# robflynnyh/long-context-asr

Measured on AMD Instinct MI355X. Metric: spectrogram-frames/sec (6L/768D, seq=16384), higher is better.
Workload: dtype bf16; 1 GPU; 6L/768D/6H SConformerXL, seq=16384, rotary theta=1.5M, fwd+CTC+bwd+clip+MADGRAD; per_gpu_batch=128, global_batch=128, seq_len=16384, parallelism=dp1

## Files before the change

long-context-asr_amd/csrc/subsample_mfma.hip:

```cpp
#include "common.h"

namespace {

constexpr int PK = 16;
constexpr int PPOS = 64;
constexpr int PATCH_BYTES = (PPOS + 1) * PK * 2;

__device__ __forceinline__ unsigned pack2(float a, float b) {
    bf16x2 t = {(bf16)a, (bf16)b};
    return __builtin_bit_cast(unsigned, t);
}
__device__ __forceinline__ float dot2(unsigned a, unsigned b, float c) {
    return __builtin_amdgcn_fdot2_f32_bf16(__builtin_bit_cast(bf16x2, a), __builtin_bit_cast(bf16x2, b), c, false);
}

template <typename TX> struct PatchEntry {
    float v0, v1;
    __device__ __forceinline__ void fetch(const TX* __restrict__ xb, int F, int T, int F2, int T2, int t2, int idx) {
        const int pos = idx >> 3, kp = idx & 7;
        const bool row_ok = t2 >= 0 && t2 < T2 && pos < F2;
        float v[2];
#pragma unroll
        for (int e = 0; e < 2; ++e) {
            const int k = 2 * kp + e, kc = min(k, 8);
            const int a = kc / 3, b = kc - 3 * a, t = 2 * t2 + a - 1, f = 2 * pos + b - 1;
            const float m = ld_f(xb + (long)min(max(f, 0), F - 1) * T + min(max(t, 0), T - 1));
            const float tap = (row_ok && t >= 0 && t < T && f >= 0 && f < F) ? m : 0.f;
            const float one = row_ok ? 1.f : 0.f;
            v[e] = k < 9 ? tap : (k < 11 ? one : 0.f);
        }
        v0 = v[0]; v1 = v[1];
    }
    __device__ __forceinline__ void store(char* patch, int idx) const {
        *reinterpret_cast<unsigned*>(patch + (idx >> 3) * (PK * 2) + (idx & 7) * 4) = pack2(v0, v1);
    }
};

__device__ __forceinline__ bf16x8 w0_frag(const float* __restrict__ w0g, const float* __restrict__ b0g, int c, int hh) {
    bf16x8 f;
    const float bias = b0g[c];
    const bf16 bh = (bf16)bias;
#pragma unroll
    for (int j = 0; j < 8; ++j) {
        const int k = 8 * hh + j;
        float v = 0.f;
        if (k < 9) v = w0g[c * 9 + min(k, 8)];
        else if (k == 9) v = (float)bh;
        else if (k == 10) v = bias - (float)bh;
        f[j] = (bf16)v;
    }
    return f;
}

template <typename TX, int NCB>
__global__ __launch_bounds__(512, (NCB == 1 ? 4 : 2)) void stage01_fwd_mfma_kernel(const TX* __restrict__ x, const float* __restrict__ w0g, const float* __restrict__ b0g,
                                                                  const float* __restrict__ wdg, const float* __restrict__ bdg, bf16* __restrict__ d1,
                                                                  int F, int T, int C, int Cs, int T2, int F2, int T4, int F4, int rows_per_block) {
    extern __shared__ __attribute__((aligned(16))) char smem[];
    const int cbase = blockIdx.z * Cs, Cl = min(Cs, C - cbase);
    w0g += cbase * 9; b0g += cbase; wdg += cbase * 9; bdg += cbase; d1 += cbase;
    const int NPAIR = F2 / 2 + 2, QS = 4 * Cl + 128, SLOT = NPAIR * QS;
    char* patch = smem;
    char* act = smem + 2 * PATCH_BYTES;
    const int tid = threadIdx.x, lane = tid & 63, wave = tid >> 6, hh = lane >> 5, cl = lane & 31;
    const int b = blockIdx.y;
    const TX* xb = x + (long)b * F * T;
    const int ncb = Cl / 32;

    bf16x8 wf[NCB];
    unsigned wj0[NCB][3][2], wj12[NCB][3][2];
    float bd2[NCB][2];
    const int cp = lane & 15, fg = lane >> 4;
#pragma unroll
    for (int u = 0; u < NCB; ++u) {
        const int cb = min(wave + 8 * u, ncb - 1);
        wf[u] = w0_frag(w0g, b0g, cb * 32 + cl, hh);
#pragma unroll
        for (int ch = 0; ch < 2; ++ch) {
            const int c = cb * 32 + 2 * cp + ch;
            bd2[u][ch] = bdg[c];
#pragma unroll
            for (int i = 0; i < 3; ++i) { wj0[u][i][ch] = pack2(0.f, wdg[c * 9 + 3 * i]); wj12[u][i][ch] = pack2(wdg[c * 9 + 3 * i + 1], wdg[c * 9 + 3 * i + 2]); }
        }
    }
    for (int i = tid; i < 3 * (QS / 4); i += 512) *reinterpret_cast<unsigned*>(act + (i / (QS / 4)) * SLOT + (i % (QS / 4)) * 4) = 0u;
    if (tid < 2 * PK / 2) *reinterpret_cast<unsigned*>(patch + (tid / (PK / 2)) * PATCH_BYTES + PPOS * PK * 2 + (tid % (PK / 2)) * 4) = 0u;

    const int r0 = blockIdx.x * rows_per_block, r1 = min(T4, r0 + rows_per_block);
    const int t2_first = 2 * r0 - 1, t2_last = 2 * (r1 - 1) + 1;
    PatchEntry<TX> pe, pe2;
    pe.fetch(xb, F, T, F2, T2, t2_first, tid);
    pe.store(patch, tid);
    pe.fetch(xb, F, T, F2, T2, t2_first + 1, tid);
    __syncthreads();
    for (int t2 = t2_first; t2 <= t2_last; ++t2) {
        const int buf = (t2 - t2_first) & 1;
        const char* pcur = patch + buf * PATCH_BYTES;
        if (t2 + 1 < t2_last) pe2.fetch(xb, F, T, F2, T2, t2 + 2, tid);
        char* arow = act + ((t2 + 3) % 3) * SLOT;
#pragma unroll
        for (int u = 0; u < NCB; ++u) {
            if (wave + 8 * u >= ncb) break;
            const int c = (wave + 8 * u) * 32 + cl;
#pragma unroll
            for (int blk = 0; blk < 2; ++blk) {
                if (blk * 32 >= F2) break;
                const bf16x8 a = *reinterpret_cast<const bf16x8*>(pcur + (blk * 32 + cl) * (PK * 2) + hh * 16);
                f32x16 acc;
#pragma unroll
                for (int r = 0; r < 16; ++r) acc[r] = 0.f;
                acc = __builtin_amdgcn_mfma_f32_32x32x16_bf16(a, wf[u], acc, 0, 0, 0);
#pragma unroll
                for (int g = 0; g < 8; ++g) {
                    const int f2 = blk * 32 + acc_row(2 * g, hh), q = (f2 + 2) >> 1;
                    if (q < NPAIR)
                        *reinterpret_cast<unsigned*>(arow + q * QS + c * 4) = pack2(siluf_(acc[2 * g]), siluf_(acc[2 * g + 1]));
                }
            }
        }
        if (t2 < t2_last) pe.store(patch + (buf ^ 1) * PATCH_BYTES, tid);
        pe = pe2;
        __syncthreads();
        if ((t2 & 1) == 0) continue;
        const int t4 = (t2 - 1) >> 1;
        if (t4 < r0) continue;
#pragma unroll
        for (int u = 0; u < NCB; ++u) {
            if (wave + 8 * u >= ncb) break;
            const int c0 = (wave + 8 * u) * 32 + 2 * cp;
#pragma unroll
            for (int fi = 0; fi < 8; ++fi) {
                const int f4 = fg + 4 * fi;
                if (f4 >= F4) break;
                float a0 = bd2[u][0], a1 = bd2[u][1];
#pragma unroll
                for (int i = 0; i < 3; ++i) {
                    const char* srow = act + ((2 * t4 + i - 1 + 3) % 3) * SLOT + c0 * 4;
                    const uint2 pa = *reinterpret_cast<const uint2*>(srow + f4 * QS);
                    const uint2 pb = *reinterpret_cast<const uint2*>(srow + (f4 + 1) * QS);
                    a0 = dot2(pa.x, wj0[u][i][0], a0); a0 = dot2(pb.x, wj12[u][i][0], a0);
                    a1 = dot2(pa.y, wj0[u][i][1], a1); a1 = dot2(pb.y, wj12[u][i][1], a1);
                }
                *reinterpret_cast<unsigned*>(d1 + (((long)b * T4 + t4) * F4 + f4) * C + c0) = pack2(a0, a1);
            }
        }
        __syncthreads();
    }
}

template <int NCB>
__global__ __launch_bounds__(512, 4) void dwconv_window_fwd_kernel(const bf16* __restrict__ x, const float* __restrict__ wdg, const float* __restrict__ bdg,
                                                                   bf16* __restrict__ y, int Ti, int Fi, int C, int To, int Fo, int rows_per_block) {
    extern __shared__ __attribute__((aligned(16))) char smem[];
    const int NPAIR = Fi / 2 + 2, QS = 4 * C + 128, SLOT = NPAIR * QS;
    char* act = smem;
    const int tid = threadIdx.x, lane = tid & 63, wave = tid >> 6;
    const int b = blockIdx.y, ncb = C / 32;
    const bf16* xb = x + (long)b * Ti * Fi * C;
    unsigned wj0[NCB][3][2], wj12[NCB][3][2];
    float bd2[NCB][2];
    const int cp = lane & 15, fg = lane >> 4;
#pragma unroll
    for (int u = 0; u < NCB; ++u) {
        const int cb = min(wave + 8 * u, ncb - 1);
#pragma unroll
        for (int ch = 0; ch < 2; ++ch) {
            const int c = cb * 32 + 2 * cp + ch;
            bd2[u][ch] = bdg[c];
#pragma unroll
            for (int i = 0; i < 3; ++i) { wj0[u][i][ch] = pack2(0.f, wdg[c * 9 + 3 * i]); wj12[u][i][ch] = pack2(wdg[c * 9 + 3 * i + 1], wdg[c * 9 + 3 * i + 2]); }
        }
    }
    for (int i = tid; i < 3 * (QS / 4); i += 512) *reinterpret_cast<unsigned*>(act + (i / (QS / 4)) * SLOT + (i % (QS / 4)) * 4) = 0u;

    const int npq = (Fi + 1) / 2, items = npq * (C / 8);
    struct Row { bf16x8 a[2], b[2]; };
    auto fetch = [&](Row& r, int ti) {
        const bool row_ok = ti >= 0 && ti < Ti;
        const bf16* src = xb + (long)min(max(ti, 0), Ti - 1) * Fi * C;
        const bf16x8 z = {0, 0, 0, 0, 0, 0, 0, 0};
#pragma unroll
        for (int it = 0; it < 2; ++it) {
            const int idx = min(tid + 512 * it, items - 1), q = idx / (C / 8), c8 = idx - q * (C / 8);
            const bf16x8 va = *reinterpret_cast<const bf16x8*>(src + (long)(2 * q) * C + c8 * 8);
            const bf16x8 vb = *reinterpret_cast<const bf16x8*>(src + (long)min(2 * q + 1, Fi - 1) * C + c8 * 8);
            r.a[it] = row_ok ? va : z;
            r.b[it] = (row_ok && 2 * q + 1 < Fi) ? vb : z;
        }
    };
    auto produce = [&](const Row& r, int ti) {
        char* arow = act + ((ti + 3) % 3) * SLOT;
#pragma unroll
        for (int it = 0; it < 2; ++it) {
            const int idx = tid + 512 * it;
            if (idx < items) {
                const int q = idx / (C / 8), c8 = idx - q * (C / 8);
                unsigned w[8];
#pragma unroll
                for (int e = 0; e < 8; ++e) w[e] = pack2(siluf_((float)r.a[it][e]), siluf_((float)r.b[it][e]));
                uint4* d = reinterpret_cast<uint4*>(arow + (q + 1) * QS + c8 * 32);
                d[0] = make_uint4(w[0], w[1], w[2], w[3]); d[1] = make_uint4(w[4], w[5], w[6], w[7]);
            }
        }
    };

    const int r0 = blockIdx.x * rows_per_block, r1 = min(To, r0 + rows_per_block);
    const int ti_first = 2 * r0 - 1, ti_last = 2 * (r1 - 1) + 1;
    Row row;
    fetch(row, ti_first);
    __syncthreads();
    for (int ti = ti_first; ti <= ti_last; ++ti) {
        produce(row, ti);
        if (ti < ti_last) fetch(row, ti + 1);
        __syncthreads();
        if ((ti & 1) == 0) continue;
        const int to = (ti - 1) >> 1;
        if (to < r0) continue;
#pragma unroll
        for (int u = 0; u < NCB; ++u) {
            if (wave + 8 * u >= ncb) break;
            const int c0 = (wave + 8 * u) * 32 + 2 * cp;
            for (int fo = fg; fo < Fo; fo += 4) {
                float a0 = bd2[u][0], a1 = bd2[u][1];
#pragma unroll
                for (int i = 0; i < 3; ++i) {
                    const char* srow = act + ((2 * to + i - 1 + 3) % 3) * SLOT + c0 * 4;
                    const uint2 pa = *reinterpret_cast<const uint2*>(srow + fo * QS);
                    const uint2 pb = *reinterpret_cast<const uint2*>(srow + (fo + 1) * QS);
                    a0 = dot2(pa.x, wj0[u][i][0], a0); a0 = dot2(pb.x, wj12[u][i][0], a0);
                    a1 = dot2(pa.y, wj0[u][i][1], a1); a1 = dot2(pb.y, wj12[u][i][1], a1);
                }
                *reinterpret_cast<unsigned*>(y + (((long)b * To + to) * Fo + fo) * C + c0) = pack2(a0, a1);
            }
        }
        __syncthreads();
    }
}

template <typename TX, int NCB>
__global__ __launch_bounds__(512, (NCB == 1 ? 4 : 2)) void stage01_bwd_mfma_kernel(const TX* __restrict__ x, const float* __restrict__ w0g, const float* __restrict__ b0g,
                                                                  const float* __restrict__ wdg, const bf16* __restrict__ dd1,
                                                                  float* __restrict__ dw0, float* __restrict__ db0, float* __restrict__ dwd, float* __restrict__ dbd,
                                                                  int F, int T, int C, int Cs, int T2, int F2, int T4, int F4, int rows_per_block,
                                                                  long det_stride) {
    extern __shared__ __attribute__((aligned(16))) char smem[];
    const int cbase = blockIdx.z * Cs, Cl = min(Cs, C - cbase);
    {
        const long drow = ((long)blockIdx.y * gridDim.x + blockIdx.x) * det_stride;
        dw0 += drow + cbase * 9; db0 += drow + cbase; dwd += drow + cbase * 9; dbd += drow + cbase;
    }
    w0g += cbase * 9; b0g += cbase; wdg += cbase * 9;
    const int GS = 2 * Cl, GSLOT = (F4 + 2) * GS;
    char* patch = smem;
    char* gimg = smem + 2 * PATCH_BYTES;
    const int tid = threadIdx.x, lane = tid & 63, wave = tid >> 6, hh = lane >> 5, cl = lane & 31;
    const int b = blockIdx.y;
    const TX* xb = x + (long)b * F * T;
    const bf16* gb = dd1 + (long)b * T4 * F4 * C + cbase;
    const int ncb = Cl / 32;

    const bool qtaps = gridDim.z > 1;
    bf16x8 wf[NCB];
    float wd[NCB][9], gwd[NCB][9], gbd[NCB];
    f32x16 aw0[NCB];
#pragma unroll
    for (int u = 0; u < NCB; ++u) {
        const int c = min(wave + 8 * u, ncb - 1) * 32 + cl;
        wf[u] = w0_frag(w0g, b0g, c, hh);
        gbd[u] = 0.f;
#pragma unroll
        for (int k = 0; k < 9; ++k) { const float w = wdg[c * 9 + k]; wd[u][k] = qtaps ? (float)(bf16)w : w; gwd[u][k] = 0.f; }
#pragma unroll
        for (int r = 0; r < 16; ++r) aw0[u][r] = 0.f;
    }
    if (tid < 2 * PK / 2) *reinterpret_cast<unsigned*>(patch + (tid / (PK / 2)) * PATCH_BYTES + PPOS * PK * 2 + (tid % (PK / 2)) * 4) = 0u;

    for (int i = tid; i < 3 * GSLOT / 4; i += 512) *reinterpret_cast<unsigned*>(gimg + i * 4) = 0u;
    __syncthreads();
    const unsigned lds_g = __builtin_amdgcn_readfirstlane(lds_addr(gimg));
    const int gseg = Cl / 8, gchunks = F4 * gseg;
    auto gissue = [&](int to) {
        if (to < 0 || to >= T4) return;
        const bf16* src = gb + (long)to * F4 * C;
        const unsigned dst = lds_g + (unsigned)((to & 1) * GSLOT) + (unsigned)__builtin_amdgcn_readfirstlane(tid & ~63) * 16u;
        for (int i = 0; i * 512 < gchunks; ++i) {
            const int ch = tid + 512 * i;
            if (ch < gchunks) dma16_asm(src + (long)(ch / gseg) * C + (ch % gseg) * 8, dst + (unsigned)(i * 512 * 16));
        }
    };

    const int r0 = blockIdx.x * rows_per_block, r1 = min(T2, r0 + rows_per_block);
    PatchEntry<TX> pe, pe2;
    pe.fetch(xb, F, T, F2, T2, r0, tid);
    gissue(r0 >> 1);
    pe.store(patch, tid);
    pe.fetch(xb, F, T, F2, T2, r0 + 1, tid);
    wait_vm<0>();
    __syncthreads();
    for (int t2 = r0; t2 < r1; ++t2) {
        const int buf = (t2 - r0) & 1;
        const char* pcur = patch + buf * PATCH_BYTES;
        const bool odd = t2 & 1;
        if (t2 + 2 < r1) pe2.fetch(xb, F, T, F2, T2, t2 + 2, tid);
        if (!odd) gissue((t2 >> 1) + 1);
        const int toX = (odd ? t2 + 1 : t2) >> 1, toZ = (t2 - 1) >> 1;
        const char* gX = gimg + (toX < T4 ? (toX & 1) : 2) * GSLOT;
        const char* gZ = gimg + (toZ & 1) * GSLOT;
#pragma unroll
        for (int u = 0; u < NCB; ++u) {
            if (wave + 8 * u >= ncb) break;
            const int c = (wave + 8 * u) * 32 + cl;
#pragma unroll 1
            for (int blk = 0; blk < 2; ++blk) {
                if (blk * 32 >= F2) break;
                const bf16x8 a = *reinterpret_cast<const bf16x8*>(pcur + (blk * 32 + cl) * (PK * 2) + hh * 16);
                f32x16 pre;
#pragma unroll
                for (int r = 0; r < 16; ++r) pre[r] = 0.f;
                pre = __builtin_amdgcn_mfma_f32_32x32x16_bf16(a, wf[u], pre, 0, 0, 0);
                unsigned dpk[8];
#pragma unroll
                for (int g4 = 0; g4 < 4; ++g4) {
                    const int base = blk * 32 + 8 * g4 + 4 * hh, p = base >> 2;
                    if (base >= F2) { dpk[2 * g4] = 0u; dpk[2 * g4 + 1] = 0u; continue; }
                    float sg[4], sv[4], gs[4];
#pragma unroll
                    for (int e = 0; e < 4; ++e) { const float v = pre[4 * g4 + e]; sg[e] = sigmoidf_(v); sv[e] = v * sg[e]; gs[e] = 0.f; }
                    auto taps = [&](const char* grow, int i) {
                        const unsigned short* gp_ = reinterpret_cast<const unsigned short*>(grow + (2 * p) * GS + c * 2);
                        const float g0 = __builtin_bit_cast(float, (unsigned)gp_[0] << 16);
                        const float g1 = __builtin_bit_cast(float, (unsigned)gp_[Cl] << 16);
                        const float g2 = __builtin_bit_cast(float, (unsigned)gp_[2 * Cl] << 16);
                        const float* w = wd[u] + 3 * i;
                        float* gw = gwd[u] + 3 * i;
                        gs[0] += w[1] * g0;                 gw[1] += g0 * sv[0];
                        gs[1] += w[0] * g1 + w[2] * g0;     gw[0] += g1 * sv[1]; gw[2] += g0 * sv[1];
                        gs[2] += w[1] * g1;                 gw[1] += g1 * sv[2];
                        gs[3] += w[0] * g2 + w[2] * g1;     gw[0] += g2 * sv[3]; gw[2] += g1 * sv[3];
                        if (i == 1) gbd[u] += g0 + g1;
                    };
                    if (!odd) taps(gX, 1);
                    else { taps(gX, 0); taps(gZ, 2); }
                    float d4[4];
#pragma unroll
                    for (int e = 0; e < 4; ++e) {
                        const float v = pre[4 * g4 + e];
                        const float d = gs[e] * sg[e] * (1.f + v * (1.f - sg[e]));
                        d4[e] = (base + e < F2) ? d : 0.f;
                    }
                    dpk[2 * g4] = pack2(d4[0], d4[1]); dpk[2 * g4 + 1] = pack2(d4[2], d4[3]);
                    __builtin_amdgcn_sched_barrier(0);
                }
                {
                    const int i16 = lane & 15, q4 = i16 >> 2, p4 = i16 & 3, G = (lane >> 4) & 1;
                    const char* tb = pcur + (blk * 32 + 4 * hh + q4) * (PK * 2) + G * 32 + (p4 >> 1) * 16 + (p4 & 1) * 8;
#pragma unroll
                    for (int half = 0; half < 2; ++half) {
                        if (blk * 32 + 16 * half >= F2) break;
                        const bf16x4 lo = __builtin_amdgcn_ds_read_tr16_b64_v4bf16((lds_p4)(tb + (16 * half) * (PK * 2)));
                        const bf16x4 hi = __builtin_amdgcn_ds_read_tr16_b64_v4bf16((lds_p4)(tb + (16 * half + 8) * (PK * 2)));
                        const bf16x8 at = __builtin_shufflevector(lo, hi, 0, 1, 2, 3, 4, 5, 6, 7);
                        const uint4 bw = make_uint4(dpk[4 * half], dpk[4 * half + 1], dpk[4 * half + 2], dpk[4 * half + 3]);
                        aw0[u] = __builtin_amdgcn_mfma_f32_32x32x16_bf16(at, __builtin_bit_cast(bf16x8, bw), aw0[u], 0, 0, 0);
                    }
                }
            }
        }
        if (t2 + 1 < r1) pe.store(patch + (buf ^ 1) * PATCH_BYTES, tid);
        pe = pe2;
        wait_vm<0>();
        __syncthreads();
    }
#pragma unroll
    for (int u = 0; u < NCB; ++u) {
        if (wave + 8 * u >= ncb) break;
        const int c = (wave + 8 * u) * 32 + cl;
#pragma unroll
        for (int r = 0; r < 4; ++r) atomicAdd(dw0 + c * 9 + 4 * hh + r, aw0[u][r]);
        if (hh == 0) { atomicAdd(dw0 + c * 9 + 8, aw0[u][4]); atomicAdd(db0 + c, aw0[u][5]); }
#pragma unroll
        for (int k = 0; k < 9; ++k) { const float v = gwd[u][k] + __shfl_xor(gwd[u][k], 32, 64); if (hh == 0) atomicAdd(dwd + c * 9 + k, v); }
        const float v = gbd[u] + __shfl_xor(gbd[u], 32, 64);
        if (hh == 0) atomicAdd(dbd + c, v);
    }
}

}

static size_t stage01_fwd_lds(int F2, long cs) { return 2 * (size_t)PATCH_BYTES + 3 * (size_t)(F2 / 2 + 2) * (4 * cs + 128); }
static size_t stage01_bwd_lds(int F4, long cs) { return 2 * (size_t)PATCH_BYTES + 3 * (size_t)(F4 + 2) * 2 * cs; }
constexpr size_t FWD_LDS_MAX = 160 * 1024, BWD_LDS_MAX = 80 * 1024;

static int stage01_slab_channels(long F, long C, bool bwd) {
    const int F2 = conv_out(F), F4 = conv_out(F2);
    if (C <= 0 || C % 32 != 0 || C > 1024 || F2 > PPOS) return 0;
    if (sub_mfma_off()) return 0;
    auto fits = [&](long cs) { return bwd ? stage01_bwd_lds(F4, cs) <= BWD_LDS_MAX : stage01_fwd_lds(F2, cs) <= FWD_LDS_MAX; };
    if (C <= 512) return fits(C) ? (int)C : 0;
    long cs = 256;
    if (const char* e = getenv("SCONF_SUB_SLAB")) { const long v = atol(e); if (v >= 32 && v <= 512 && v % 32 == 0) cs = v; }
    while (cs > 32 && !fits(cs)) cs -= 32;
    return fits(cs) ? (int)cs : 0;
}
int stage01_mfma_slabs(int64_t F, int64_t C, int bwd) {
    const int cs = stage01_slab_channels(F, C, bwd != 0);
    return cs ? (int)cdiv(C, (long)cs) : 0;
}

int sconf_stage01_fwd_mfma(const void* x, int x_dtype, const float* w0, const float* b0, const float* wd, const float* bd, void* d1,
                           int64_t B, int64_t F, int64_t T, int64_t C, hipStream_t stream) {
    const int T2 = conv_out(T), F2 = conv_out(F), T4 = conv_out(T2), F4 = conv_out(F2);
    const int Cs = stage01_slab_channels(F, C, false);
    if (!Cs) return 0;
    const size_t sh = stage01_fwd_lds(F2, Cs);
    const long target = env_long("SCONF_SUB_FWD_BLOCKS", 4096);
    const int rpb = std::max(1, (int)cdiv((long)T4 * B, target));
    dim3 grid(cdiv(T4, rpb), (unsigned)B, (unsigned)cdiv(C, (long)Cs)), block(512);
#define LF(TX, NCB_) do { \
        static bool attr = false; lds_limit_once(attr, {(const void*)stage01_fwd_mfma_kernel<TX, NCB_>}, FWD_LDS_MAX); \
        hipLaunchKernelGGL((stage01_fwd_mfma_kernel<TX, NCB_>), grid, block, sh, stream, (const TX*)x, w0, b0, wd, bd, (bf16*)d1, (int)F, (int)T, (int)C, Cs, T2, F2, T4, F4, rpb); } while (0)
    if (x_dtype == SCONF_F32) { if (Cs <= 256) LF(float, 1); else LF(float, 2); }
    else                      { if (Cs <= 256) LF(bf16, 1); else LF(bf16, 2); }
#undef LF
    return 1;
}

static bool stage01_bwd_mfma_geo(long B, long F, long T, long C, dim3& grid, size_t& sh, int& rpb, int& Cs) {
    const int T2 = conv_out(T), F2 = conv_out(F), F4 = conv_out(F2);
    Cs = stage01_slab_channels(F, C, true);
    if (!Cs) return false;
    sh = stage01_bwd_lds(F4, Cs);
    const long target = env_long("SCONF_SUB_BWD_BLOCKS", 2048);
    rpb = std::max(2, (int)cdiv((long)T2 * B, target));
    rpb += rpb & 1;
    grid = dim3(cdiv(T2, rpb), (unsigned)B, (unsigned)cdiv(C, (long)Cs));
    return true;
}
int64_t stage01_bwd_mfma_workspace(int64_t B, int64_t F, int64_t T, int64_t C) {
    dim3 grid; size_t sh; int rpb, Cs;
    if (B * T * F == 0 || !stage01_bwd_mfma_geo(B, F, T, C, grid, sh, rpb, Cs)) return 0;
    return (int64_t)grid.x * grid.y * 20 * C * 4;
}

int sconf_stage01_bwd_mfma(const void* dd1, const void* x, int x_dtype, const float* w0, const float* b0, const float* wd,
                           float* dw0, float* db0, float* dwd, float* dbd, void* workspace, int64_t workspace_bytes,
                           int64_t B, int64_t F, int64_t T, int64_t C, hipStream_t stream) {
    const int T2 = conv_out(T), F2 = conv_out(F), T4 = conv_out(T2), F4 = conv_out(F2);
    dim3 grid; size_t sh; int rpb, Cs;
    if (!stage01_bwd_mfma_geo(B, F, T, C, grid, sh, rpb, Cs)) return 0;
    const dim3 block(512);
    const long rows = (long)grid.x * grid.y, dst = 20 * C;
    float* sl = det_begin<float>(workspace, workspace_bytes, rows, dst, stream);
    if (!sl) { sconf_set_error("sconf_sub_stage01_bwd: needs %ld bytes of workspace (sconf_sub_stage01_bwd_workspace)", rows * dst * 4); return -1; }
#define LB(TX, NCB_) do { \
        if (sh > 64 * 1024) { static bool attr = false; lds_limit_once(attr, {(const void*)stage01_bwd_mfma_kernel<TX, NCB_>}, BWD_LDS_MAX); } \
        hipLaunchKernelGGL((stage01_bwd_mfma_kernel<TX, NCB_>), grid, block, sh, stream, (const TX*)x, w0, b0, wd, (const bf16*)dd1, sl, sl + 9 * C, sl + 10 * C, sl + 19 * C, (int)F, (int)T, (int)C, Cs, T2, F2, T4, F4, rpb, dst); } while (0)
    if (x_dtype == SCONF_F32) { if (Cs <= 256) LB(float, 1); else LB(float, 2); }
    else                      { if (Cs <= 256) LB(bf16, 1); else LB(bf16, 2); }
#undef LB
    det_finish<float>(sl, rows, dst, DetSegs<float>{{dw0, db0, dwd, dbd}, {0, 9 * C, 10 * C, 19 * C}, {9 * C, C, 9 * C, C}, 4}, stream);
    return 1;
}

int sconf_dwconv_window_fwd(const void* x, const float* w, const float* bias, void* y, int64_t B, int64_t Ti, int64_t Fi, int64_t C, hipStream_t stream) {
    const int To = conv_out(Ti), Fo = conv_out(Fi);
    if (C % 32 != 0 || C > 512 || ((Fi + 1) / 2) * (C / 8) > 1024) return 0;
    if (sub_mfma_off()) return 0;
    const size_t sh = 3 * (size_t)(Fi / 2 + 2) * (4 * C + 128);
    if (sh > 160 * 1024) return 0;
    const long target = env_long("SCONF_SUB_FWD_BLOCKS", 4096);
    const int rpb = std::max(1, (int)cdiv((long)To * B, target));
    dim3 grid(cdiv(To, rpb), (unsigned)B), block(512);
#define LW(NCB_) do { \
        static bool attr = false; lds_limit_once(attr, {(const void*)dwconv_window_fwd_kernel<NCB_>}, 160 * 1024); \
        hipLaunchKernelGGL((dwconv_window_fwd_kernel<NCB_>), grid, block, sh, stream, (const bf16*)x, w, bias, (bf16*)y, (int)Ti, (int)Fi, (int)C, To, Fo, rpb); } while (0)
    if (C <= 256) LW(1); else LW(2);
#undef LW
    return 1;
}
```

Before: 7.124 million spectrogram-frames/sec.

## Batch patch fetches by R rows and per-wave dd1 DMA layout in subsample bwd

The stage0/1 backward kernel now fetches input patches for R conv0 rows at once into a double set of R patch buffers. It synchronises once per group instead of once per row, with a partial vmcnt wait so the dd1 DMA for the next row can stay in flight. The gradient image in LDS is changed to per-wave 32-channel bins so each wave issues its own DMA, and patch fetches now keep raw inputs in registers and convert them at store time. The kernel also gains optional timestamp instrumentation, and the LDS footprint grows with R.

```diff
diff --git a/long-context-asr_amd/csrc/subsample_mfma.hip b/long-context-asr_amd/csrc/subsample_mfma.hip
--- a/long-context-asr_amd/csrc/subsample_mfma.hip
+++ b/long-context-asr_amd/csrc/subsample_mfma.hip
@@ -1,6 +1,29 @@
+#ifdef SCONF_SUB_STAMP
+#define SCONF_STAMPS
+#endif
 #include "common.h"
 
 namespace {
+
+#ifdef SCONF_SUB_STAMP
+__device__ unsigned long long g_sub_stamps[2 * 8 * 8];
+#define STAMP_OUT(k) do { if (blockIdx.x == gridDim.x / 2 && blockIdx.y == gridDim.y / 2 && blockIdx.z == 0 && (threadIdx.x & 63) == 0) \
+        for (int i_ = 0; i_ < 8; ++i_) g_sub_stamps[((k) * 8 + (threadIdx.x >> 6)) * 8 + i_] = st_acc_[i_]; } while (0)
+static void sub_stamp_print(int k, double rows, hipStream_t stream, const char* legend) {
+    if (!getenv("SCONF_SUB_STAMP_PRINT")) return;
+    (void)hipStreamSynchronize(stream);
+    unsigned long long h[2 * 8 * 8];
+    (void)hipMemcpyFromSymbol(h, HIP_SYMBOL(g_sub_stamps), sizeof(h));
+    for (int w = 0; w < 8; ++w) {
+        fprintf(stderr, "[stage01 %s stamps] wave %d:", k ? "bwd" : "fwd", w);
+        double tot = 0;
+        for (int i = 0; i < 8; ++i) { fprintf(stderr, " %7.1f", (double)h[(k * 8 + w) * 8 + i] / rows); tot += (double)h[(k * 8 + w) * 8 + i] / rows; }
+        fprintf(stderr, "  sum %7.1f   (memtime ticks per conv0 row over %.0f rows: %s)\n", tot, rows, legend);
+    }
+}
+#else
+#define STAMP_OUT(k)
+#endif
 
 constexpr int PK = 16;
 constexpr int PPOS = 64;
@@ -15,26 +38,39 @@
 }
 
 template <typename TX> struct PatchEntry {
-    float v0, v1;
-    __device__ __forceinline__ void fetch(const TX* __restrict__ xb, int F, int T, int F2, int T2, int t2, int idx) {
-        const int pos = idx >> 3, kp = idx & 7;
-        const bool row_ok = t2 >= 0 && t2 < T2 && pos < F2;
+    TX r0, r1;
+    int t2;
+    static __device__ __forceinline__ void tap_of(int t2, int idx, int e, int& k, int& t, int& f) {
+        k = 2 * (idx & 7) + e;
+        const int kc = min(k, 8), a = kc / 3, b = kc - 3 * a;
+        t = 2 * t2 + a - 1; f = 2 * (idx >> 3) + b - 1;
+    }
+    __device__ __forceinline__ void fetch(const TX* __restrict__ xb, int F, int T, int t2_, int idx) {
+        int k, t, f;
+        t2 = t2_;
+        tap_of(t2, idx, 0, k, t, f); r0 = xb[(long)min(max(f, 0), F - 1) * T + min(max(t, 0), T - 1)];
+        tap_of(t2, idx, 1, k, t, f); r1 = xb[(long)min(max(f, 0), F - 1) * T + min(max(t, 0), T - 1)];
+    }
+    __device__ __forceinline__ void store(char* patch, int F, int T, int F2, int T2, int idx) const {
+        const bool row_ok = t2 >= 0 && t2 < T2 && (idx >> 3) < F2;
         float v[2];
 #pragma unroll
         for (int e = 0; e < 2; ++e) {
-            const int k = 2 * kp + e, kc = min(k, 8);
-            const int a = kc / 3, b = kc - 3 * a, t = 2 * t2 + a - 1, f = 2 * pos + b - 1;
-            const float m = ld_f(xb + (long)min(max(f, 0), F - 1) * T + min(max(t, 0), T - 1));
+            int k, t, f;
+            tap_of(t2, idx, e, k, t, f);
+            const float m = (float)(e ? r1 : r0);
             const float tap = (row_ok && t >= 0 && t < T && f >= 0 && f < F) ? m : 0.f;
             const float one = row_ok ? 1.f : 0.f;
             v[e] = k < 9 ? tap : (k < 11 ? one : 0.f);
         }
-        v0 = v[0]; v1 = v[1];
-    }
-    __device__ __forceinline__ void store(char* patch, int idx) const {
-        *reinterpret_cast<unsigned*>(patch + (idx >> 3) * (PK * 2) + (idx & 7) * 4) = pack2(v0, v1);
+        *reinterpret_cast<unsigned*>(patch + (idx >> 3) * (PK * 2) + (idx & 7) * 4) = pack2(v[0], v[1]);
     }
 };
+
+__device__ __forceinline__ float dp_of(float gs, float sg, float pre) {
+#pragma clang fp reassociate(off)
+    return ((1.f + pre * (1.f - sg)) * sg) * gs;
+}
 
 __device__ __forceinline__ bf16x8 w0_frag(const float* __restrict__ w0g, const float* __restrict__ b0g, int c, int hh) {
     bf16x8 f;
@@ -89,14 +125,16 @@
     const int r0 = blockIdx.x * rows_per_block, r1 = min(T4, r0 + rows_per_block);
     const int t2_first = 2 * r0 - 1, t2_last = 2 * (r1 - 1) + 1;
     PatchEntry<TX> pe, pe2;
-    pe.fetch(xb, F, T, F2, T2, t2_first, tid);
-    pe.store(patch, tid);
-    pe.fetch(xb, F, T, F2, T2, t2_first + 1, tid);
+    pe.fetch(xb, F, T, t2_first, tid);
+    pe.store(patch, F, T, F2, T2, tid);
+    pe.fetch(xb, F, T, t2_first + 1, tid);
     __syncthreads();
+    STAMP_DECL(8)
     for (int t2 = t2_first; t2 <= t2_last; ++t2) {
         const int buf = (t2 - t2_first) & 1;
         const char* pcur = patch + buf * PATCH_BYTES;
-        if (t2 + 1 < t2_last) pe2.fetch(xb, F, T, F2, T2, t2 + 2, tid);
+        if (t2 + 1 < t2_last) pe2.fetch(xb, F, T, t2 + 2, tid);
+        STAMP(0);
         char* arow = act + ((t2 + 3) % 3) * SLOT;
 #pragma unroll
         for (int u = 0; u < NCB; ++u) {
@@ -118,9 +156,12 @@
                 }
             }
         }
-        if (t2 < t2_last) pe.store(patch + (buf ^ 1) * PATCH_BYTES, tid);
+        STAMP(2);
+        if (t2 < t2_last) pe.store(patch + (buf ^ 1) * PATCH_BYTES, F, T, F2, T2, tid);
         pe = pe2;
+        STAMP(3);
         __syncthreads();
+        STAMP(5);
         if ((t2 & 1) == 0) continue;
         const int t4 = (t2 - 1) >> 1;
         if (t4 < r0) continue;
@@ -144,8 +185,11 @@
                 *reinterpret_cast<unsigned*>(d1 + (((long)b * T4 + t4) * F4 + f4) * C + c0) = pack2(a0, a1);
             }
         }
+        STAMP(6);
         __syncthreads();
-    }
+        STAMP(7);
+    }
+    STAMP_OUT(0);
 }
 
 template <int NCB>
@@ -237,7 +281,7 @@
     }
 }
 
-template <typename TX, int NCB>
+template <typename TX, int NCB, int R>
 __global__ __launch_bounds__(512, (NCB == 1 ? 4 : 2)) void stage01_bwd_mfma_kernel(const TX* __restrict__ x, const float* __restrict__ w0g, const float* __restrict__ b0g,
                                                                   const float* __restrict__ wdg, const bf16* __restrict__ dd1,
                                                                   float* __restrict__ dw0, float* __restrict__ db0, float* __restrict__ dwd, float* __restrict__ dbd,
@@ -250,9 +294,11 @@
         dw0 += drow + cbase * 9; db0 += drow + cbase; dwd += drow + cbase * 9; dbd += drow + cbase;
     }
     w0g += cbase * 9; b0g += cbase; wdg += cbase * 9;
-    const int GS = 2 * Cl, GSLOT = (F4 + 2) * GS;
+    static_assert(R >= 2 && R % 2 == 0, "a group starts on an even conv0 row");
+    const int GBIN = 64, GCB = (F4 + 2) * GBIN;
+    const int GSLOT = (Cl / 32) * GCB;
     char* patch = smem;
-    char* gimg = smem + 2 * PATCH_BYTES;
+    char* gimg = smem + 2 * R * PATCH_BYTES;
     const int tid = threadIdx.x, lane = tid & 63, wave = tid >> 6, hh = lane >> 5, cl = lane & 31;
     const int b = blockIdx.y;
     const TX* xb = x + (long)b * F * T;
@@ -273,43 +319,59 @@
 #pragma unroll
         for (int r = 0; r < 16; ++r) aw0[u][r] = 0.f;
     }
-    if (tid < 2 * PK / 2) *reinterpret_cast<unsigned*>(patch + (tid / (PK / 2)) * PATCH_BYTES + PPOS * PK * 2 + (tid % (PK / 2)) * 4) = 0u;
+    if (tid < 2 * R * (PK / 2)) *reinterpret_cast<unsigned*>(patch + (tid / (PK / 2)) * PATCH_BYTES + PPOS * PK * 2 + (tid % (PK / 2)) * 4) = 0u;
 
     for (int i = tid; i < 3 * GSLOT / 4; i += 512) *reinterpret_cast<unsigned*>(gimg + i * 4) = 0u;
     __syncthreads();
     const unsigned lds_g = __builtin_amdgcn_readfirstlane(lds_addr(gimg));
-    const int gseg = Cl / 8, gchunks = F4 * gseg;
+    const int wave_u = __builtin_amdgcn_readfirstlane(wave);
+    const int gpieces = 4 * F4;
     auto gissue = [&](int to) {
         if (to < 0 || to >= T4) return;
-        const bf16* src = gb + (long)to * F4 * C;
-        const unsigned dst = lds_g + (unsigned)((to & 1) * GSLOT) + (unsigned)__builtin_amdgcn_readfirstlane(tid & ~63) * 16u;
-        for (int i = 0; i * 512 < gchunks; ++i) {
-            const int ch = tid + 512 * i;
-            if (ch < gchunks) dma16_asm(src + (long)(ch / gseg) * C + (ch % gseg) * 8, dst + (unsigned)(i * 512 * 16));
+#pragma unroll
+        for (int u = 0; u < NCB; ++u) {
+            if (wave_u + 8 * u >= ncb) break;
+            const bf16* src = gb + (long)to * F4 * C + (wave_u + 8 * u) * 32;
+            const unsigned dst = lds_g + (unsigned)((to & 1) * GSLOT + (wave_u + 8 * u) * GCB);
+            for (int i = 0; i * 64 < gpieces; ++i) {
+                const int ch = lane + 64 * i;
+                if (ch < gpieces) dma16_asm(src + (long)(ch >> 2) * C + (ch & 3) * 8, dst + (unsigned)(i * 64 * 16));
+            }
         }
     };
 
     const int r0 = blockIdx.x * rows_per_block, r1 = min(T2, r0 + rows_per_block);
-    PatchEntry<TX> pe, pe2;
-    pe.fetch(xb, F, T, F2, T2, r0, tid);
+    PatchEntry<TX> pe[R];
+#pragma unroll
+    for (int j = 0; j < R; ++j) pe[j].fetch(xb, F, T, r0 + j, tid);
     gissue(r0 >> 1);
-    pe.store(patch, tid);
-    pe.fetch(xb, F, T, F2, T2, r0 + 1, tid);
+#pragma unroll
+    for (int j = 0; j < R; ++j) pe[j].store(patch + j * PATCH_BYTES, F, T, F2, T2, tid);
     wait_vm<0>();
     __syncthreads();
+    STAMP_DECL(8)
     for (int t2 = r0; t2 < r1; ++t2) {
-        const int buf = (t2 - r0) & 1;
-        const char* pcur = patch + buf * PATCH_BYTES;
+        const int j = (t2 - r0) % R, set = ((t2 - r0) / R) & 1;
+        const char* pcur = patch + (set * R + j) * PATCH_BYTES;
         const bool odd = t2 & 1;
-        if (t2 + 2 < r1) pe2.fetch(xb, F, T, F2, T2, t2 + 2, tid);
-        if (!odd) gissue((t2 >> 1) + 1);
+        const bool more = t2 - j + R < r1;
+        if (!odd && t2 + 1 < r1) gissue((t2 >> 1) + 1);
+        STAMP(1);
+        if (j == 0 && more) {
+#pragma unroll
+            for (int jj = 0; jj < R; ++jj) pe[jj].fetch(xb, F, T, t2 + R + jj, tid);
+        }
+        STAMP(0);
+        if (odd) {
+            if (j == 1 && more) wait_vm<2 * R>(); else wait_vm<0>();
+        }
+        STAMP(4);
         const int toX = (odd ? t2 + 1 : t2) >> 1, toZ = (t2 - 1) >> 1;
         const char* gX = gimg + (toX < T4 ? (toX & 1) : 2) * GSLOT;
         const char* gZ = gimg + (toZ & 1) * GSLOT;
 #pragma unroll
         for (int u = 0; u < NCB; ++u) {
             if (wave + 8 * u >= ncb) break;
-            const int c = (wave + 8 * u) * 32 + cl;
 #pragma unroll 1
             for (int blk = 0; blk < 2; ++blk) {
                 if (blk * 32 >= F2) break;
@@ -327,10 +389,10 @@
 #pragma unroll
                     for (int e = 0; e < 4; ++e) { const float v = pre[4 * g4 + e]; sg[e] = sigmoidf_(v); sv[e] = v * sg[e]; gs[e] = 0.f; }
                     auto taps = [&](const char* grow, int i) {
-                        const unsigned short* gp_ = reinterpret_cast<const unsigned short*>(grow + (2 * p) * GS + c * 2);
+                        const unsigned short* gp_ = reinterpret_cast<const unsigned short*>(grow + (wave + 8 * u) * GCB + (2 * p) * GBIN + cl * 2);
                         const float g0 = __builtin_bit_cast(float, (unsigned)gp_[0] << 16);
-                        const float g1 = __builtin_bit_cast(float, (unsigned)gp_[Cl] << 16);
-                        const float g2 = __builtin_bit_cast(float, (unsigned)gp_[2 * Cl] << 16);
+                        const float g1 = __builtin_bit_cast(float, (unsigned)gp_[GBIN / 2] << 16);
+                        const float g2 = __builtin_bit_cast(float, (unsigned)gp_[GBIN] << 16);
                         const float* w = wd[u] + 3 * i;
                         float* gw = gwd[u] + 3 * i;
                         gs[0] += w[1] * g0;                 gw[1] += g0 * sv[0];
@@ -345,7 +407,7 @@
 #pragma unroll
                     for (int e = 0; e < 4; ++e) {
                         const float v = pre[4 * g4 + e];
-                        const float d = gs[e] * sg[e] * (1.f + v * (1.f - sg[e]));
+                        const float d = dp_of(gs[e], sg[e], v);
                         d4[e] = (base + e < F2) ? d : 0.f;
                     }
                     dpk[2 * g4] = pack2(d4[0], d4[1]); dpk[2 * g4 + 1] = pack2(d4[2], d4[3]);
@@ -366,11 +428,19 @@
                 }
             }
         }
-        if (t2 + 1 < r1) pe.store(patch + (buf ^ 1) * PATCH_BYTES, tid);
-        pe = pe2;
-        wait_vm<0>();
-        __syncthreads();
-    }
+        STAMP(2);
+        if (j == R - 1 || t2 + 1 == r1) {
+            if (more) {
+#pragma unroll
+                for (int jj = 0; jj < R; ++jj) pe[jj].store(patch + ((set ^ 1) * R + jj) * PATCH_BYTES, F, T, F2, T2, tid);
+            }
+            STAMP(3);
+            wait_lgkm0_barrier();
+            STAMP(5);
+        }
+    }
+    wait_vm<0>();
+    STAMP_OUT(1);
 #pragma unroll
     for (int u = 0; u < NCB; ++u) {
         if (wave + 8 * u >= ncb) break;
@@ -388,7 +458,7 @@
 }
 
 static size_t stage01_fwd_lds(int F2, long cs) { return 2 * (size_t)PATCH_BYTES + 3 * (size_t)(F2 / 2 + 2) * (4 * cs + 128); }
-static size_t stage01_bwd_lds(int F4, long cs) { return 2 * (size_t)PATCH_BYTES + 3 * (size_t)(F4 + 2) * 2 * cs; }
+static size_t stage01_bwd_lds(int F4, long cs, int R = 2) { return 2 * R * (size_t)PATCH_BYTES + 3 * (size_t)(F4 + 2) * 2 * cs; }
 constexpr size_t FWD_LDS_MAX = 160 * 1024, BWD_LDS_MAX = 80 * 1024;
 
 static int stage01_slab_channels(long F, long C, bool bwd) {
@@ -422,6 +492,9 @@
     if (x_dtype == SCONF_F32) { if (Cs <= 256) LF(float, 1); else LF(float, 2); }
     else                      { if (Cs <= 256) LF(bf16, 1); else LF(bf16, 2); }
 #undef LF
+#ifdef SCONF_SUB_STAMP
+    sub_stamp_print(0, 2.0 * rpb + 1, stream, "patch fetch issue, -, conv0 MFMA + SiLU + window store, patch store, -, barrier 1, depthwise row (per conv0 row), barrier 2");
+#endif
     return 1;
 }
 
@@ -452,12 +525,15 @@
     const long rows = (long)grid.x * grid.y, dst = 20 * C;
     float* sl = det_begin<float>(workspace, workspace_bytes, rows, dst, stream);
     if (!sl) { sconf_set_error("sconf_sub_stage01_bwd: needs %ld bytes of workspace (sconf_sub_stage01_bwd_workspace)", rows * dst * 4); return -1; }
-#define LB(TX, NCB_) do { \
-        if (sh > 64 * 1024) { static bool attr = false; lds_limit_once(attr, {(const void*)stage01_bwd_mfma_kernel<TX, NCB_>}, BWD_LDS_MAX); } \
-        hipLaunchKernelGGL((stage01_bwd_mfma_kernel<TX, NCB_>), grid, block, sh, stream, (const TX*)x, w0, b0, wd, (const bf16*)dd1, sl, sl + 9 * C, sl + 10 * C, sl + 19 * C, (int)F, (int)T, (int)C, Cs, T2, F2, T4, F4, rpb, dst); } while (0)
-    if (x_dtype == SCONF_F32) { if (Cs <= 256) LB(float, 1); else LB(float, 2); }
-    else                      { if (Cs <= 256) LB(bf16, 1); else LB(bf16, 2); }
+#define LB(TX, NCB_, R_) do { \
+        if (sh > 64 * 1024) { static bool attr = false; lds_limit_once(attr, {(const void*)stage01_bwd_mfma_kernel<TX, NCB_, R_>}, BWD_LDS_MAX); } \
+        hipLaunchKernelGGL((stage01_bwd_mfma_kernel<TX, NCB_, R_>), grid, block, sh, stream, (const TX*)x, w0, b0, wd, (const bf16*)dd1, sl, sl + 9 * C, sl + 10 * C, sl + 19 * C, (int)F, (int)T, (int)C, Cs, T2, F2, T4, F4, rpb, dst); } while (0)
+    if (x_dtype == SCONF_F32) { if (Cs <= 256) LB(float, 1, 2); else LB(float, 2, 2); }
+    else                      { if (Cs <= 256) LB(bf16, 1, 2); else LB(bf16, 2, 2); }
 #undef LB
+#ifdef SCONF_SUB_STAMP
+    sub_stamp_print(1, rpb, stream, "patch fetch issue, dd1 DMA issue, MFMA + taps + elementwise, patch store, vmcnt wait, barrier, -, -");
+#endif
     det_finish<float>(sl, rows, dst, DetSegs<float>{{dw0, db0, dwd, dbd}, {0, 9 * C, 10 * C, 19 * C}, {9 * C, C, 9 * C, C}, 4}, stream);
     return 1;
 }
```

Measured after the change: 7.140 million spectrogram-frames/sec (median of 4 runs). Within noise of the previous version (+0.2%).
